# byteowlz/kokorox

Measured on AMD Instinct MI355X. Metric: real-time factor (audio-s/wall-s), 24 kHz, batch=64, higher is better.
Workload: dtype f32 in / out, f32 accumulate; products on split operands: f16f8 (a_hi b_hi on f16 MFMAs, the cross terms a_lo b_hi + a_hi b_lo of the 7 / 11-tap convs on e4m3 scaled MFMAs: ~17 significant bits per product; every other conv f16x3: ~22) -- wider than the bf16 BASELINE configs[2] names, inside the 1e-; 1 GPU; batch=64/GPU synthetic 128-phoneme utterances (T=130), durations pinned 3,3,3,4 -> F=422 frames = 10.55 s each, noise on, inputs in HBM; batch_per_gpu=64, frames=422, parallelism=utterance-sharded x1, one-time weight broadcast

## Files before the change

kokorox_amd/build.py:

```python
from __future__ import annotations

import os
import subprocess
import sys

HERE = os.path.dirname(os.path.abspath(__file__))
CSRC = os.path.join(HERE, "csrc")
LIB_DIR = os.path.join(HERE, "lib")
LIB_PATH = os.path.join(LIB_DIR, "libkokorox_hip.so")
TEST_LIB_PATH = os.path.join(LIB_DIR, "libkokorox_hip_test.so")
TEST_SOURCES = ["test_hooks.hip"]
SOURCES = ["conv_plan.hip", "conv_call.hip", "conv_mfma.hip", "conv_f16x3.hip", "conv_f16x3_da.hip", "conv_f16x3_da_p1.hip", "conv_f16x3_da_w2.hip", "conv_f16x3_da_s16.hip", "conv_f16x3_da_f8.hip", "conv_f16x3_da_pre.hip", "conv_f16x3_pre.hip", "conv_f16x3_dapn.hip", "conv_f16x3_dag.hip", "kernels_misc.hip", "request_kernels.hip", "model.hip", "model_forward.hip", "model_host.hip", "api.hip", "dispatcher.hip", "onnx_import.cpp", "kxw_file.cpp",
           "host_request.cpp", "host_pool.cpp"]
HEADERS = ["kx_common.h", "kx_error.h", "host_request.h", "conv_epilogue.h", "conv_f16x3_common.h"]
_PUB = os.path.join("..", "..", "include", "kokorox_hip.h")
_PUB_TEST = os.path.join("..", "..", "include", "kokorox_hip_test.h")
_MODEL_H = ["model.h", "kxw_file.h", "onnx_import.h"]
EXTRA_DEPS = {"model.hip": [*_MODEL_H, _PUB], "model_forward.hip": [*_MODEL_H, _PUB], "model_host.hip": [*_MODEL_H, "host_pool.h", _PUB],
              "host_pool.cpp": ["host_pool.h"], "host_request.cpp": ["resample_taps.h", "kweight_coefs.h", "truepeak_taps.h"], "request_kernels.hip": ["resample_taps.h", "kweight_coefs.h", "truepeak_taps.h"], "conv_call.hip": _MODEL_H, "api.hip": [*_MODEL_H, "kx_handle.h", "api_guard.h", "check_device.h", _PUB],
              "dispatcher.hip": [*_MODEL_H, "kx_handle.h", "dispatcher_core.h", _PUB],
              "test_hooks.hip": [*_MODEL_H, "kx_handle.h", "api_guard.h", "check_device.h", _PUB, _PUB_TEST], "onnx_import.cpp": ["onnx_import.h"],
              "kxw_file.cpp": ["kxw_file.h", "onnx_import.h"], "conv_f16x3_da_p1.hip": ["conv_f16x3_da.hip"], "conv_f16x3_da_w2.hip": ["conv_f16x3_da.hip"], "conv_f16x3_da_s16.hip": ["conv_f16x3_da.hip"], "conv_f16x3_da_f8.hip": ["conv_f16x3_da.hip"], "conv_f16x3_da_pre.hip": ["conv_f16x3_da.hip"]}
FLAGS = ["-O3", "--offload-arch=gfx950", "-fPIC", "-std=c++17", "-Wall", "-Wno-unused-result"]


def _hipcc() -> str:
    for cand in (os.environ.get("HIPCC"), "/opt/rocm/bin/hipcc", "hipcc"):
        if cand and (os.path.isabs(cand) and os.path.exists(cand) or not os.path.isabs(cand)):
            return cand
    return "hipcc"


def _newer(target: str, deps) -> bool:
    if not os.path.exists(target):
        return False
    t = os.path.getmtime(target)
    return all(os.path.getmtime(d) <= t for d in deps)


LAST_BUILD = {"compiled": [], "reused": [], "linked": False}


def build_library(force: bool = False, verbose: bool = False) -> str:
    LAST_BUILD["compiled"], LAST_BUILD["reused"], LAST_BUILD["linked"] = [], [], False
    os.makedirs(LIB_DIR, exist_ok=True)
    hdrs = [os.path.join(CSRC, h) for h in HEADERS]
    objs, test_objs, jobs = [], [], []
    for src in SOURCES + TEST_SOURCES:
        s = os.path.join(CSRC, src)
        o = os.path.join(LIB_DIR, os.path.splitext(src)[0] + ".o")
        (test_objs if src in TEST_SOURCES else objs).append(o)
        if force or not _newer(o, [s] + hdrs + [os.path.join(CSRC, d) for d in EXTRA_DEPS.get(src, [])]):
            flags = [f for f in FLAGS if not f.startswith("--offload-arch")] if src.endswith(".cpp") else FLAGS
            jobs.append([_hipcc(), *flags, "-c", s, "-o", o])
            LAST_BUILD["compiled"].append(src)
        else:
            LAST_BUILD["reused"].append(src)
    if jobs:
        from concurrent.futures import ThreadPoolExecutor

        def run(cmd):
            if verbose:
                print(" ".join(cmd), file=sys.stderr)
            subprocess.run(cmd, check=True)

        with ThreadPoolExecutor(max_workers=min(4, len(jobs))) as ex:
            list(ex.map(run, jobs))
    if force or not _newer(LIB_PATH, objs):
        cmd = [_hipcc(), "--offload-arch=gfx950", "-shared", "-fPIC", *objs, "-lpthread", "-o", LIB_PATH]
        if verbose:
            print(" ".join(cmd), file=sys.stderr)
        subprocess.run(cmd, check=True)
        LAST_BUILD["linked"] = True
    if force or not _newer(TEST_LIB_PATH, test_objs + [LIB_PATH]):
        cmd = [_hipcc(), "--offload-arch=gfx950", "-shared", "-fPIC", *test_objs, "-L" + LIB_DIR, "-lkokorox_hip", "-Wl,-rpath,$ORIGIN",
               "-lpthread", "-o", TEST_LIB_PATH]
        if verbose:
            print(" ".join(cmd), file=sys.stderr)
        subprocess.run(cmd, check=True)
    return LIB_PATH


if __name__ == "__main__":
    print(build_library(force="--force" in sys.argv, verbose=True))
```

kokorox_amd/csrc/conv_f16x3.hip:

```cpp
#include "conv_f16x3_common.h"

namespace kx {

template <int BM, int BN, int WM, int WN, int ACT, int TK, bool PF, int VT>
__global__ __launch_bounds__(WM * WN * 64, (WM * WN == 8) ? 4 : ((BM / WM / 32) * (BN / WN / 32) > 6 ? 2 : 3))
void conv1d_f16x3_kernel(const ConvArgs a) {
    constexpr int MT = BM / WM / 32;
    constexpr int NT = BN / WN / 32;
    constexpr int NWV = WM * WN;
    static_assert((NWV == 4 || NWV == 8) && MT >= 1 && NT >= 1, "4 or 8 waves per workgroup");
    static_assert(VT == 1 || (VT <= TK && PF), "virtual taps need TK >= VT and the prefetching build");
    extern __shared__ __attribute__((aligned(16))) unsigned char smem16[];

    const int tid = threadIdx.x;
    const int lane = tid & 63;
    const int wave = __builtin_amdgcn_readfirstlane(tid >> 6);
    const int wm = wave / WN, wn = wave % WN;
    const int r = lane & 31, h = lane >> 5;
    const int b = blockIdx.z, ct = blockIdx.y;
    int tile_x = blockIdx.x;
    if (a.xcd_swizzle && gridDim.x >= 16) {
        const int nx = gridDim.x;
        const int off = (int)(((long)nx * (blockIdx.y + (long)gridDim.y * blockIdx.z)) & 7);
        const int cls = (blockIdx.x + off) & 7;
// ... 300 lines not shown

template <int BM, int BN, int WM, int WN, int ACT, int TK, bool PF, int VT = 1>
static void launch_inst16_pf(const ConvArgs& a, int B, int max_cols, hipStream_t s) {
    static DynLdsLimit lds_limit;
    auto kern = conv1d_f16x3_kernel<BM, BN, WM, WN, ACT, TK, PF, VT>;
    const int XW = (BN - 1) * a.stride + (a.K - 1) * a.dil + 1;
    const int XWp = PF ? ((VT > 1) ? 128 : BN + 128) : ((XW + 3) & ~3);
    KX_REQUIRE(!PF || (a.stride == 1 && XW <= XWp), "conv1d f16x3: the prefetching build needs stride 1 and a window <= BN + 128");
    const size_t lds = 16 * ((size_t)2 * TK * 4 * BM + (size_t)VT * 4 * XWp);
    KX_REQUIRE(lds <= 160 * 1024, "conv1d f16x3: LDS tile too large for this k/stride");
    KX_REQUIRE(VT == 1 || (a.K == 1 && a.stride == 1 && XW <= 128), "conv1d f16x3: virtual taps need a k=1 GEMM");
    lds_limit.ensure(reinterpret_cast<const void*>(kern), lds);
    dim3 grid((max_cols + BN - 1) / BN, (a.Cout + BM - 1) / BM, a.merge_T > 0 ? 1 : B);
    KX_REQUIRE(grid.x > 0 && grid.y > 0 && grid.y < 65536 && B > 0 && B < 65536, "conv1d f16x3: bad grid");
    KX_REQUIRE(a.merge_T == 0 || (PF && a.K == 1 && a.stride == 1 && a.pad == 0 && !a.in_up2 && !a.nmean &&
                                  a.store != ST_UPSCATTER && !a.stat_part),
               "conv1d f16x3: merged columns need a plain k=1 GEMM");
    hipLaunchKernelGGL(kern, grid, dim3(WM * WN * 64), lds, s, a);
    KX_HIP(hipGetLastError());
}

template <int BM, int BN, int WM, int WN, int ACT>
static void launch_inst16_act(const ConvPlan& p, const ConvArgs& a, int B, hipStream_t s) {
    if (p.pf)
        launch_inst16_pf<BM, BN, WM, WN, ACT, 3, true>(a, B, p.cols, s);
    else
        launch_inst16_pf<BM, BN, WM, WN, ACT, 3, false>(a, B, p.cols, s);
}

template <int BM, int BN, int WM, int WN>
static void launch_inst16(const ConvPlan& p, const ConvArgs& a, int B, hipStream_t s) {
    if (p.act == ACT_SNAKE)
        launch_inst16_act<BM, BN, WM, WN, ACT_SNAKE>(p, a, B, s);
    else if (p.act == ACT_LEAKY)
        launch_inst16_act<BM, BN, WM, WN, ACT_LEAKY>(p, a, B, s);
    else
        launch_inst16_act<BM, BN, WM, WN, ACT_NONE>(p, a, B, s);
}

static void launch_lds(const ConvPlan& p, const ConvArgs& a, int B, hipStream_t s) {
    if (p.vt > 1) {
        KX_REQUIRE(p.bm == 128 && p.bn == 128 && p.pf && p.act != ACT_SNAKE && (p.vt == 2 || p.vt == 3), "conv1d f16x3: no such virtual-tap form");
        if (p.vt == 3) {
            if (p.act == ACT_LEAKY)
                launch_inst16_pf<128, 128, 2, 2, ACT_LEAKY, 3, true, 3>(a, B, p.cols, s);
            else
                launch_inst16_pf<128, 128, 2, 2, ACT_NONE, 3, true, 3>(a, B, p.cols, s);
        } else {
            if (p.act == ACT_LEAKY)
                launch_inst16_pf<128, 128, 2, 2, ACT_LEAKY, 2, true, 2>(a, B, p.cols, s);
            else
                launch_inst16_pf<128, 128, 2, 2, ACT_NONE, 2, true, 2>(a, B, p.cols, s);
        }
        return;
    }
    const int bm = p.bm, bn = p.bn, wm = p.wm, wn = p.wn;
    if (bm == 128 && bn == 128 && wm == 4 && wn == 1)
        launch_inst16<128, 128, 4, 1>(p, a, B, s);
    else if (bm == 128 && bn == 128 && wm == 2 && wn == 2)
        launch_inst16<128, 128, 2, 2>(p, a, B, s);
    else if (bm == 128 && bn == 256 && wm == 2 && wn == 2)
        launch_inst16<128, 256, 2, 2>(p, a, B, s);
    else if (bm == 64 && bn == 256 && wm == 1 && wn == 4)
        launch_inst16<64, 256, 1, 4>(p, a, B, s);
    else if (bm == 32 && bn == 256 && wm == 1 && wn == 4)
        launch_inst16<32, 256, 1, 4>(p, a, B, s);
    else
        throw Error(1, "conv1d f16x3: no such LDS-DMA form");
}

void launch_conv(const ConvPlan& p, const ConvArgs& a, int B, hipStream_t s) {
    if (p.form == FORM_F32) {
        launch_conv1d(a, p.bm, B, p.cols, s);
        return;
    }
    KX_REQUIRE(a.n_chunks16 == (a.Cin + CK16 - 1) / CK16 && a.w16 != nullptr, "conv1d f16x3: weights not packed");
    KX_REQUIRE(a.epi != EPI_GELU_NEW || p.vt > 1 || p.form == FORM_DAG || p.form == FORM_DAGN,
               "conv1d f16x3: gelu epilogue exists only for k=1 GEMMs with >= 48 input channels");
    KX_REQUIRE(p.merged == (a.merge_T > 0), "conv1d f16x3: merged columns do not match the plan");
    if (p.cols <= 0) return;
    switch (p.form) {
        case FORM_LDS: launch_lds(p, a, B, s); return;
        case FORM_DAG:
        case FORM_DAGN: launch_conv1d_f16x3_dag(p, a, B, s); return;
        case FORM_DAPN: launch_conv1d_f16x3_dapn(a, B, p.cols, s); return;
        case FORM_DA_PRE: launch_conv16_da_pre(p, a, B, s); return;
        case FORM_DA_S16: launch_conv16_da_s16(p, a, B, s); return;
        case FORM_DA_F8: launch_conv16_da_f8(p, a, B, s); return;
        case FORM_DA:
            if (p.p1) {
                launch_conv16_da_p1(p, a, B, s);
                return;
            }
            [[fallthrough]];
        case FORM_DA_W2:
            if (p.form == FORM_DA_W2)
                launch_conv16_da_w2(p, a, B, s);
            else
                launch_conv16_da(p, a, B, s);
            return;
    }
    throw Error(1, "conv1d: unknown kernel form");
}

size_t packed_conv16_halves(int rows, int Cin, int K, int BM) {
    const size_t tiles = (rows + BM - 1) / BM, chunks = (Cin + CK16 - 1) / CK16;
    return tiles * chunks * K * 4 * BM * 8;
}

__global__ void absmax_kernel(const float* p, long n, unsigned* out) {
    unsigned m = 0u;
    for (long i = blockIdx.x * (long)blockDim.x + threadIdx.x; i < n; i += (long)gridDim.x * blockDim.x) {
        const unsigned u = __float_as_uint(p[i]) & 0x7fffffffu;
        m = u > m ? u : m;
    }
    for (int o = 32; o > 0; o >>= 1) {
        const unsigned u = (unsigned)__shfl_down((int)m, o);
        m = u > m ? u : m;
    }
    if ((threadIdx.x & 63) == 0) atomicMax(out, m);
}

float device_absmax(const float* p, long n, hipStream_t s) {
    unsigned* d;
    KX_HIP(hipMalloc((void**)&d, 4));
    KX_HIP(hipMemsetAsync(d, 0, 4, s));
    const int blocks = (int)((n + 255) / 256 < 1024 ? (n + 255) / 256 : 1024);
    hipLaunchKernelGGL(absmax_kernel, dim3(blocks), dim3(256), 0, s, p, n, d);
    unsigned hbits = 0;
    KX_HIP(hipMemcpyAsync(&hbits, d, 4, hipMemcpyDeviceToHost, s));
    KX_HIP(hipStreamSynchronize(s));
    KX_HIP(hipFree(d));
    float f;
    memcpy(&f, &hbits, 4);
    return f;
}

int pick_weight_shift(float absmax) {
    if (!(absmax > 0.f) || !std::isfinite(absmax)) return 0;
    int e;
    frexpf(absmax, &e);
    int ws = 12 - e;
    if (ws < -8) ws = -8;
    if (ws > 24) ws = 24;
    return ws;
}

__global__ void pack_conv16_kernel(PackSrc src, _Float16* dst, int Cout, int Cin, int K, int BM, float wscale,
                                   long total_pairs) {
    const int n_chunks = (Cin + CK16 - 1) / CK16;
    for (long e = blockIdx.x * (long)blockDim.x + threadIdx.x; e < total_pairs; e += (long)gridDim.x * blockDim.x) {
        long q = e;
        const int j8 = q % 8; q /= 8;
        const int m = q % BM; q /= BM;
        const int hh = q % 2; q /= 2;
        const int tap = q % K; q /= K;
        const int ch = q % n_chunks; q /= n_chunks;
        const int co = (int)q * BM + m, ci = ch * CK16 + hh * 8 + j8;
        float v = 0.f;
        if (co < Cout && ci < Cin) {
            int rr = co;
            const float* p = src.p[0];
            if (rr >= src.rows[0]) { rr -= src.rows[0]; p = src.p[1];
                if (rr >= src.rows[1]) { rr -= src.rows[1]; p = src.p[2]; } }
            v = p[((long)rr * Cin + ci) * K + tap] * wscale;
        }
// ... 109 lines not shown
```

kokorox_amd/csrc/conv_plan.hip:

```cpp
#include "kx_common.h"

namespace kx {

static bool da_eligible(int BM, int K, int dil, int stride, bool merged) {
    return BM == 128 && stride == 1 && !merged && (K - 1) * dil + 256 <= 384;
}

static bool f8_taps(int K, int dil) { return (K == 11 || K == 7 || K == 3) && (K - 1) * dil <= 64; }

static bool s16_shape(int BM, int K, int dil, int stride, int act, int n_chunks16, bool merged, int pmode) {
    const bool taps = K == 11 || (K == 7 && dil == 1) || (pmode == 2 && f8_taps(K, dil));
    return BM == 128 && stride == 1 && !merged && pmode != 1 && act == ACT_SNAKE && taps && (K - 1) * dil <= 64 && n_chunks16 >= 2 &&
           (n_chunks16 & 1) == 0;
}

bool conv16_f8_layer(int BM, int rows, int K, int n_chunks16) {
    return BM == 128 && f8_taps(K, 1) && (K != 3 || rows <= 256) && n_chunks16 >= 2 && (n_chunks16 & 1) == 0;
}

ConvPlan conv_plan(const ConvLaunch& c) {
    ConvPlan p{};
    p.bm = c.BM;
    p.act = c.act;
    p.vt = 1;
    p.cols = c.cols;
    const bool stats = c.stats && c.store == ST_NORMAL && !c.accum;
    auto set_stats = [&](int stat_cols) {
        if (!stats) return;
        p.stat_cols = stat_cols;
        p.stat_tiles = (p.cols + p.bn - 1) / p.bn * (p.bn / stat_cols);
    };
    if (c.mode == CONV_F32) {
        p.form = FORM_F32;
        p.bn = c.BM == 128 ? 128 : 256;
        set_stats(64);
        return p;
    }
    const int route = c.force & 3;
    const int pmode = c.prec1 ? 1 : (c.f8 ? 2 : 0);

    const bool pre_form = c.stride == 1 && c.K >= 2 && !c.in_up2 && c.act != ACT_SNAKE && !c.prec1 &&
                          da_eligible(c.BM, c.K, c.dil, c.stride, false);
    p.pre = (c.mode == CONV_F16X3 || c.mode == CONV_F16F8) && c.image && pre_form && (c.image == 2 || c.rows >= 512);

    p.merged = c.B > 1 && c.K == 1 && c.stride == 1 && c.pad == 0 && !c.in_up2 && !c.norm && c.store != ST_UPSCATTER && !c.stats &&
               c.merge_T > 0 && c.merge_T <= 512;
    if (p.merged) p.cols = c.B * c.merge_T;

    if (c.BM != 128) {
        p.form = FORM_LDS;
        p.bn = 256;
        p.wm = 1;
        p.wn = 4;
        p.pf = c.stride == 1 && (c.K - 1) * c.dil <= 128;
        set_stats(64);
        return p;
    }

    if (c.K == 1 && c.stride == 1 && !stats && !c.in_up2 && c.n_chunks16 >= 3 && c.act != ACT_SNAKE) {
        const long tiles = (long)((p.cols + 127) / 128) * ((c.rows + 127) / 128);
        if (route != FORCE_LDS && !c.norm && c.store != ST_UPSCATTER) {
            const long wgs = tiles * (p.merged ? 1 : c.B);
            const bool narrow_ok = (c.x_bs * c.B + 16L * c.x_ld) * 4 < (1L << 31);
            p.form = narrow_ok && 2 * wgs <= c.cus ? FORM_DAGN : FORM_DAG;
            p.bn = p.form == FORM_DAGN ? 32 : 128;
            return p;
        }
        p.form = FORM_LDS;
        p.bn = 128;
        p.wm = 2;
        p.wn = 2;
        p.pf = 1;
        p.vt = tiles > 2L * c.cus ? 2 : 3;
        return p;
    }

    const bool da = route != FORCE_LDS && da_eligible(c.BM, c.K, c.dil, c.stride, p.merged);
    const bool small = (long)((p.cols + 255) / 256) * ((c.rows + 127) / 128) * c.B < 256;
    if (route != FORCE_LDS && !(c.force & FORCE_NO_S16) && s16_shape(c.BM, c.K, c.dil, c.stride, c.act, c.n_chunks16, p.merged, pmode)) {
        p.form = pmode == 2 ? FORM_DA_F8 : FORM_DA_S16;
        p.kt = c.K;
        p.bn = small && route != FORCE_DA ? 128 : 192;
        set_stats(64);
    } else if (!da || (route != FORCE_DA && c.cols <= 160 && !stats)) {
        p.form = FORM_LDS;
        const bool short_seq = c.cols <= 160 && !stats;
        p.bn = !short_seq && !small ? 256 : 128;
        p.wm = !short_seq && small ? 4 : 2;
        p.wn = !short_seq && small ? 1 : 2;
        p.pf = c.stride == 1 && (c.K - 1) * c.dil <= 128;
        set_stats(p.bn / p.wn);
    } else {
        p.bn = small && route != FORCE_DA ? 128 : 256;
        set_stats(128);
        const bool w64 = (c.K - 1) * c.dil <= 64;
        if (p.pre) {
            const bool narrow = p.bn == 128 && !c.prec1 && c.rows % 32 == 0 && c.K <= 12 && c.epi == EPI_NONE &&
                                (c.store == ST_NORMAL || c.store == ST_UPSCATTER) && (long)c.n_chunks16 * c.K < 5000;
            p.form = narrow ? FORM_DAPN : FORM_DA_PRE;
            p.act = ACT_NONE;
            p.kt = c.K == 3 && w64 ? 3 : 0;
        } else {
            const bool unrolled = w64 && ((c.act == ACT_SNAKE && (c.K == 11 || c.K == 7 || c.K == 3)) || (c.act == ACT_LEAKY && c.K == 3));
            p.kt = unrolled ? c.K : 0;
            p.p1 = c.prec1 != 0;
            p.bf = c.prec1 == 2;
            p.form = unrolled && p.bn == 256 && !c.prec1 && !(c.force & FORCE_DA_4X1) ? FORM_DA_W2 : FORM_DA;
        }
    }
    const bool flat_form = p.form != FORM_LDS;
    p.flat_bn = flat_form && c.B > 1 && p.cols > 0 ? p.bn : 0;
    return p;
}

}
```

kokorox_amd/csrc/kx_common.h:

```cpp
#pragma once
#include <hip/hip_runtime.h>

#include <cmath>
#include <cstdint>
#include <cstring>
#include <cstdio>
#include <stdexcept>
#include <string>
#include <vector>

#include <atomic>
#include <mutex>

#include "host_request.h"
#include "kx_error.h"

namespace kx {

constexpr int KX_MAX_DEVICES = 64;

struct DynLdsLimit {
    std::atomic<size_t> limit[KX_MAX_DEVICES];
    std::mutex mu;
    DynLdsLimit() {
// ... 21 lines not shown

struct LenMap {
    const int* lens;
    int mul, add;
};

constexpr int CONV_CK = 8;

enum ConvAct { ACT_NONE = 0, ACT_LEAKY = 1, ACT_SNAKE = 2 };
enum ConvStore { ST_NORMAL = 0, ST_TMAJOR = 1, ST_UPSCATTER = 2 };
enum ConvEpi { EPI_NONE = 0, EPI_GELU_NEW = 1 };

struct ConvArgs {
    const float* x;
    long x_bs;
    int x_ld;
    int Cin;
    LenMap in_len;
    LenMap out_len;
    const float* w;
    const float* bias;
    const float* nmean;
    const float* nscale;
    const float* nshift;
    int n_bs;
    int act;
    float slope;
    const float* alpha;
    int K, dil, stride, pad;
    int in_up2;
    int Cout;
    int n_chunks;
    float* y;
    long y_bs;
    int y_ld;
    const float* resid;
    long r_bs;
    int r_ld;
    int accum;
    float out_mul;
    float out_div;
    int epi;
    int store;
    int up_s, up_pad, up_off, up_reflect, up_cout;
    const void* w16;
    const void* w16b;
    const void* w8x;
    int epi_stream;
    int n_chunks16;
    float w_unscale;
    float x_prescale;
    int merge_T;
    int merge_B;
    float2* stat_part;
    int stat_tiles;
    int xcd_swizzle;
    int ws_force;
    unsigned long long* stamps;
    int prec1;
    int dephase_cycles, dephase_mode;
    int dbg;
    const int* tile_prefix;
    int flat_ny;
    int flat_B;
    int flat_tiles_host, flat_bn_host;
    const void* x16;
    long x16_bs;
    int x16_ld;
};

enum ConvMode { CONV_F32 = 0, CONV_F16X3 = 1, CONV_F16X3_LDS = 2, CONV_F16X3_DA = 3, CONV_F16 = 4, CONV_BF16 = 5, CONV_F16F8 = 6 };
enum ConvForm {
    FORM_F32 = 0,
    FORM_LDS,
    FORM_DAG,
    FORM_DAGN,
    FORM_DA,
    FORM_DA_W2,
    FORM_DA_S16,
    FORM_DA_F8,
    FORM_DA_PRE,
    FORM_DAPN,
};
enum ConvForce { FORCE_LDS = 1, FORCE_DA = 2, FORCE_DA_4X1 = 4, FORCE_NO_S16 = 8 };

struct ConvLaunch {
    int mode;
    int prec1;
    int f8;
    int BM, rows, n_chunks16, K, dil, stride, pad, act, in_up2, store, accum, epi;
    int norm;
    int stats;
    int image;
    int merge_T;
    long x_bs;
    int x_ld;
    int B, cols;
    int cus;
    int force;
};
struct ConvPlan {
    int form;
    int bm, act, kt, wm, wn, vt, pf, p1, bf;
    int bn;
    int cols;
    int merged;
    int pre;
    int stat_cols, stat_tiles;
    int flat_bn;
};
ConvPlan conv_plan(const ConvLaunch& c);
bool conv16_f8_layer(int BM, int rows, int K, int n_chunks16);
void launch_conv(const ConvPlan& p, const ConvArgs& a, int B, hipStream_t s);
int conv16_cu_count();
int cu_count_override();

size_t conv16_pre_image_bytes(int Cin, int x_ld);
void launch_split_image(const ConvArgs& a, int B, int Lmax, void* img, long img_bs, hipStream_t s);

void launch_tile_prefix(LenMap len, int extra, int bn, int B, int* out, hipStream_t s);

inline int conv_pick_bm(int rows) { return rows >= 128 ? 128 : (rows > 32 ? 64 : 32); }

void launch_conv1d(const ConvArgs& a, int BM, int B, int max_cols, hipStream_t s);

struct PackSrc {
    const float* p[3];
    int rows[3];
};
void launch_pack_conv(const PackSrc& src, float* dst, int Cout, int Cin, int K, int BM, hipStream_t s);
void launch_pack_convT(const float* w, float* dst, int Cin, int Cout, int s, int BM, hipStream_t s_);
size_t packed_conv_floats(int rows, int Cin, int K, int BM);

void launch_conv16_da(const ConvPlan& p, const ConvArgs& a, int B, hipStream_t s);
void launch_conv16_da_p1(const ConvPlan& p, const ConvArgs& a, int B, hipStream_t s);
void launch_conv16_da_w2(const ConvPlan& p, const ConvArgs& a, int B, hipStream_t s);
void launch_conv16_da_s16(const ConvPlan& p, const ConvArgs& a, int B, hipStream_t s);
void launch_conv16_da_f8(const ConvPlan& p, const ConvArgs& a, int B, hipStream_t s);
void launch_conv16_da_pre(const ConvPlan& p, const ConvArgs& a, int B, hipStream_t s);
void launch_conv1d_f16x3_dapn(const ConvArgs& a, int B, int max_cols, hipStream_t s);
void launch_conv1d_f16x3_dag(const ConvPlan& p, const ConvArgs& a, int B, hipStream_t s);
size_t packed_conv16_halves(int rows, int Cin, int K, int BM);
float device_absmax(const float* p, long n, hipStream_t s);
int pick_weight_shift(float absmax);
void launch_pack_conv16(const PackSrc& src, void* dst, int Cout, int Cin, int K, int BM, float wscale, hipStream_t s);
void launch_pack_convT16(const float* w, void* dst, int Cin, int Cout, int sd, int BM, float wscale, hipStream_t s);
void launch_image_to_bf16(const void* w16, void* dst, size_t n_halves, hipStream_t s);
size_t packed_conv8x_bytes(int rows, int Cin, int K);
void launch_pack_conv8x(const void* w16, void* dst, int rows, int Cin, int K, hipStream_t s);

void launch_vec_add(const float* a, const float* b, float* out, int n, hipStream_t s);
void launch_transpose_whh(const float* whh, float* out, hipStream_t s);

void launch_albert_embed(const int64_t* ids, long ids_stride, const float* word, const float* type0,
                         const float* pos, float* out, long bs, int ld, const int* lens, int B, int Tmax,
                         int n_vocab, unsigned* bad_id, hipStream_t s);
void launch_embed(const int64_t* ids, long ids_stride, const float* table, int C, float* out, long bs, int ld,
                  const int* lens, int B, int Tmax, int n_vocab, unsigned* bad_id, hipStream_t s);

enum LnMode { LN_PLAIN = 0, LN_AFFINE = 1, LN_ADA = 2 };
void launch_layernorm_ch(const float* x, float* y, long bs, int ld, int C, LenMap len, int B, int Lmax,
                         float eps, int mode, const float* g, const float* be, int g_bs, float leaky,
                         hipStream_t s);

void launch_attention(const float* qkv, long bs, int ld, float* ctx, long cbs, int cld, const int* lens, int B,
                      int Tmax, hipStream_t s);

struct FcDesc {
    const float* w;
    const float* b;
    int n_out;
    int style_off;
    long out_off;
};
void launch_style_fc(const FcDesc* d_desc, int n_desc, const float* styles, float* out, long out_bs, int B,
                     hipStream_t s);

constexpr int STAT_RAW_TILES = 0;
void launch_stats_finalize(const float2* part, int tiles, int cols_per_tile, int C, LenMap len, int B, const float* gb,
                           long gb_bs, float* mean, float* scale, float* shift, int n_bs, hipStream_t s);
void launch_in_stats(const float* x, long bs, int ld, int C, LenMap len, int B, const float* gb, long gb_bs,
                     float* mean, float* scale, float* shift, int n_bs, float2* raw_out, hipStream_t s);

void launch_diag_stats(const float* x, long bs, int ld, int C, LenMap len, int B, int Lmax, const float* nmean,
                       const float* nscale, const float* nshift, int n_bs, float* out3, hipStream_t s);

void launch_style_mix(const float* table, int n_voices, const int* voice_ids, const float* weights, int max_mix,
                      const int* rows, const int* kinds, float* styles, int B, hipStream_t s);

struct OutputTables {
    PackReq* req;
    long* cum;
    JoinRow* join;
    MarkRow* mark;
    LevelSpec* level;
    uint32_t* peak;
    LoudSpec* loud;
    double* hops;
    double* loud_pow;
    uint32_t* tpeak;
};
void launch_output_plan(const float* audio, long audio_ld, const int* dur, const int* lens, const OutputPlan& plan,
                        const OutputTables& t, float* d_y, void* d_packed, hipStream_t s);
void launch_pack_plan(const float* audio, long audio_ld, const OutputPlan& plan, const OutputTables& t, float* d_y, void* out,
                      hipStream_t s);
void launch_token_marks(const int* dur, const int* lens, const OutputPlan& plan, const OutputTables& t, void* marks, hipStream_t s);
void launch_edge_durations(const int* dur, const int* lens, int* edges, int B, hipStream_t s);
void* host_out_alloc(size_t bytes);
void host_out_free(void* p);
void host_out_share(void* base, void* const* parts, int n);
size_t host_out_live_bytes();
void launch_fill_style_rows(float* dst, long bs, int ld, int row0, const float* styles, int style_off,
                            const int* lens, int B, int Tmax, hipStream_t s);
void launch_copy_rows(const float* src, long sbs, int sld, float* dst, long dbs, int dld, int rows, LenMap len,
                      int B, int Lmax, hipStream_t s);

void launch_lstm(const float* gx, long gx_bs, int gx_ld, const float* whhT, float* y, long y_bs, int y_ld,
                 LenMap len, int B, unsigned long long* xchg, unsigned* err_word, hipStream_t s,
                 unsigned* epoch_state = nullptr);
size_t lstm_exchange_bytes(int B);
void lstm_set_parts(int n);
void lstm_set_test_fault(int on);

void launch_duration(const float* logits, long bs, int ld, const float* speeds, int n_speed, const int* lens,
// ... 23 lines not shown
```

kokorox_amd/hip_koko.py:

```python
from __future__ import annotations

import ctypes as C
import os
from typing import List, Optional, Sequence

import numpy as np

_HERE = os.path.dirname(os.path.abspath(__file__))
LIB_PATH = os.path.join(_HERE, "lib", "libkokorox_hip.so")

PACK_F32_MONO, PACK_F32_STEREO, PACK_PCM16_MONO = 0, 1, 2
PACK_WAV_F32, PACK_WAV16_BASE64 = 3, 4
PACK_MULAW, PACK_ALAW = 8, 9
PACK_RATE_24000, PACK_RATE_8000, PACK_RATE_16000, PACK_RATE_48000 = 0x000, 0x100, 0x200, 0x300
RATE_HZ = {0: 24000, 1: 8000, 2: 16000, 3: 48000}
RESAMPLE_MAX_TAPS = 145
JOIN_TRIM_HEAD, JOIN_TRIM_TAIL, JOIN_TRIM_INNER = 1, 2, 4
JOIN_DTYPE = np.dtype([("flags", "<u4"), ("keep_ms", "<i4"), ("pause_ms", "<i4"), ("fade_ms", "<i4")])
JOIN_NONE = (0, 0, 0, 0)
LEVEL_GAIN, LEVEL_NORMALIZE, LEVEL_CEILING = 0, 1, 2
LEVEL_DTYPE = np.dtype([("mode", "<u4"), ("gain", "<f4"), ("peak", "<f4")])
LEVEL_PLAIN = (LEVEL_GAIN, 1.0, 0.0)
PEAK_TRUE = 0x100
LOUDNESS_MEASURE, LOUDNESS_NORMALIZE = 0, 1
# ... 761 lines not shown
        try:
            raw = C.string_at(out, nb.value)
            if marks:
                if (mk.value or 0) % 8 != 0 or (mk.value or 0) < out.value + nb.value:
                    raise KokoroxHipError(3, "marks are not 8-byte aligned behind the body")
                m = np.frombuffer(C.string_at(mk, 8 * n_mk.value), dtype=np.int64).copy()
        finally:
            self._lib.kx_free_packed(out)
        res = (_decode_packed(raw, fmt), m) if marks else (_decode_packed(raw, fmt),)
        res = res + (lv_out,) if level is not None else res
        res = res + (ld_out,) if loudness is not None else res
        return res if len(res) > 1 else res[0]

    def stats(self):
        a, b, c = C.c_int64(0), C.c_int64(0), C.c_int64(0)
        self._lib.kx_dispatcher_stats(self._d, C.byref(a), C.byref(b), C.byref(c))
        per = (C.c_int64 * len(self._models))()
        self._lib.kx_dispatcher_model_batches(self._d, per, len(self._models))
        rp, rt = C.c_int64(0), C.c_int64(0)
        self._lib.kx_dispatcher_failures(self._d, C.byref(rp), C.byref(rt))
        hl = (C.c_int32 * len(self._models))()
        mf, rq = C.c_int64(0), C.c_int64(0)
        self._lib.kx_dispatcher_health(self._d, hl, len(self._models), C.byref(mf), C.byref(rq))
        return {"requests": a.value, "batches": b.value, "max_batch": c.value, "batches_per_model": list(per),
                "replayed_requests": rp.value, "retried_batches": rt.value, "healthy": [int(v) for v in hl],
                "failed_models": mf.value, "requeued_requests": rq.value}

    def close(self):
        if getattr(self, "_d", None):
            self._lib.kx_dispatcher_destroy(self._d)
            self._d = None

    def __del__(self):
        try:
            self.close()
        except Exception:
            pass


def import_onnx(onnx_path: str, out_path: str) -> str:
    lib = load_library()
    err = C.create_string_buffer(2048)
    rc = lib.kx_import_onnx(os.fsencode(onnx_path), os.fsencode(out_path), err, len(err))
    if rc != KX_OK:
        raise KokoroxHipError(rc, err.value.decode(errors="replace"))
    return out_path


def _err_call(fn, *args):
    err = C.create_string_buffer(512)
    rc = fn(*args, err, len(err))
    if rc != 0:
        raise KokoroxHipError(rc, err.value.decode())


CONV_F32, CONV_F16X3, CONV_F16F8 = 0, 1, 6
STFT_ONNX, STFT_TORCH = 0, 1


def conv1d(x, w, bias=None, stride=1, pad=0, dil=1, transposed=False, act=0, slope=0.0, alpha=None, norm=None,
           device=0, mode=None, pre=False):
    lib = load_test_library()
    if mode is None:
        mode = CONV_F32 if os.environ.get("KOKOROX_CONV", "") == "f32" else CONV_F16X3
    x, w = _f32(x), _f32(w)
    B, Cin, L = x.shape
    k = w.shape[2]
    if transposed:
        Cout = w.shape[1]
        Lout = (L - 1) * stride - 2 * pad + k
    else:
        Cout = w.shape[0]
        Lout = (L + 2 * pad - dil * (k - 1) - 1) // stride + 1
    y = np.zeros((B, Cout, Lout), dtype=np.float32)
    bias, alpha, norm = _f32(bias), _f32(alpha), _f32(norm)
    _err_call(lib.kx_test_conv1d, device, _ptr(x), B, Cin, L, _ptr(w), _ptr(bias), Cout, k, stride, pad, dil,
              1 if transposed else 0, act, float(slope), _ptr(alpha), _ptr(norm), _ptr(y), Lout, mode | (0x100 if pre else 0))
    return y


CONV_LAUNCH_FIELDS = ("mode", "prec1", "f8", "BM", "rows", "n_chunks16", "K", "dil", "stride", "pad", "act", "in_up2", "store", "accum",
                      "epi", "norm", "stats", "image", "merge_T", "x_bs", "x_ld", "B", "cols", "cus", "force")
CONV_PLAN_FIELDS = ("form", "bm", "act", "kt", "wm", "wn", "vt", "pf", "p1", "bf", "bn", "cols", "merged", "pre", "stat_cols",
                    "stat_tiles", "flat_bn")
CONV_FORMS = ("F32", "LDS", "DAG", "DAGN", "DA", "DA_W2", "DA_S16", "DA_F8", "DA_PRE", "DAPN")


def conv_plan(**launch):
    lib = load_test_library()
    unknown = set(launch) - set(CONV_LAUNCH_FIELDS)
    assert not unknown, unknown
    src = np.array([int(launch.get(f, 0)) for f in CONV_LAUNCH_FIELDS], dtype=np.int64)
    out = np.zeros(len(CONV_PLAN_FIELDS), dtype=np.int64)
    _err_call(lib.kx_test_conv_plan, _ptr(src), len(src), _ptr(out), len(out))
    plan = dict(zip(CONV_PLAN_FIELDS, (int(v) for v in out)))
    plan["form"] = CONV_FORMS[plan["form"]]
    return plan


def conv_transpose(x, w, bias=None, stride=6, act=1, slope=0.1, resid=None, up_off=0, mode=1, pre=False, device=0):
    lib = load_test_library()
    x, w = _f32(x), _f32(w)
    B, Cin, L = x.shape
    Cout, k = w.shape[1], w.shape[2]
    assert k == 2 * stride
    pad = (k - stride) // 2
    Lout = (L - 1) * stride - 2 * pad + k
    y = np.zeros((B, Cout, Lout + (1 if up_off else 0)), dtype=np.float32)
    _err_call(lib.kx_test_conv_transpose, device, _ptr(x), B, Cin, L, _ptr(w), _ptr(_f32(bias)), Cout, stride, act, float(slope),
              _ptr(_f32(resid)), 1 if up_off else 0, _ptr(y), mode | (0x100 if pre else 0))
    return y


def conv1d_epilogue(x, w, bias=None, pad=0, dil=1, resid=None, y_init=None, out_mul=1.0, out_div=1.0, want_stats=False,
                    mode=1, device=0):
    lib = load_test_library()
    x, w = _f32(x), _f32(w)
    B, Cin, L = x.shape
    Cout, _, k = w.shape
    Lout = L + 2 * pad - dil * (k - 1)
    y = np.zeros((B, Cout, Lout), dtype=np.float32) if y_init is None else _f32(y_init).copy()
    st = np.zeros((B, Cout, 2), dtype=np.float32) if want_stats else None
    _err_call(lib.kx_test_conv1d_epilogue, device, _ptr(x), B, Cin, L, _ptr(w), _ptr(_f32(bias)), Cout, k, pad, dil,
              _ptr(_f32(resid)), 0 if y_init is None else 1, float(out_mul), float(out_div), _ptr(y), _ptr(st), mode)
    return (y, st) if want_stats else y


def conv1d_full(x, w, bias=None, pad=0, dil=1, act=0, slope=0.0, alpha=None, norm=None, resid=None, y_init=None,
                out_mul=1.0, out_div=1.0, want_stats=False, lens=None, pad_ld=False, flat=False, mode=1, device=0, pre=False):
    lib = load_test_library()
    x, w = _f32(x), _f32(w)
    B, Cin, L = x.shape
    Cout, _, k = w.shape
    Lout = L + 2 * pad - dil * (k - 1)
    y = np.zeros((B, Cout, Lout), dtype=np.float32) if y_init is None else _f32(y_init).copy()
    st = np.zeros((B, Cout, 2), dtype=np.float32) if want_stats else None
    ln = None if lens is None else np.ascontiguousarray(lens, dtype=np.int32)
    _err_call(lib.kx_test_conv1d_full, device, _ptr(x), B, Cin, L, _ptr(ln), (1 if pad_ld else 0) | (2 if flat else 0), _ptr(w), _ptr(_f32(bias)),
              Cout, k, pad, dil, act, float(slope), _ptr(_f32(alpha)), _ptr(_f32(norm)), _ptr(_f32(resid)),
              0 if y_init is None else 1, float(out_mul), float(out_div), _ptr(y), _ptr(st), mode | (0x100 if pre else 0))
    return (y, st) if want_stats else y


def conv1d_opts(x, w, bias=None, pad=0, dil=1, act=0, slope=0.0, alpha=None, norm=None, resid=None, y_init=None,
                out_mul=1.0, out_div=1.0, want_stats=False, lens=None, pad_ld=False, flat=False, mode=1, device=0, pre=False,
                in_up2=False, epi=0, merged=False, tmajor=False, prec1=0, act_shift=0, epi_stream=False, want_norm=None,
                up_stride=0, stride=1, len_in=None, len_out=None, up_off=False, view=False):
    lib = load_test_library()
    x, w = _f32(x), _f32(w)
    B, Cin, L = x.shape
    Cout, _, k = w.shape
    Lout = ((2 * L if in_up2 else L) + 2 * pad - dil * (k - 1) - 1) // stride + 1
    if up_stride:
        Cout = w.shape[1]
        assert k == 2 * up_stride
        Lout = (L - 1) * up_stride - 2 * ((k - up_stride) // 2) + k + (1 if up_off else 0)
    shape = (B, Lout, Cout) if tmajor else (B, Cout, Lout)
    y = np.zeros(shape, dtype=np.float32) if y_init is None else _f32(y_init).copy()
    st = np.zeros((B, Cout, 2), dtype=np.float32) if want_stats else None
    ln = None if lens is None else np.ascontiguousarray(lens, dtype=np.int32)
    opts = [in_up2, epi, merged, tmajor, prec1, act_shift, epi_stream, up_stride]
    if stride != 1 or len_in is not None or len_out is not None or up_off or view:
        opts += [stride, *(len_in or (0, 0)), *(len_out or (0, 0)), up_off, view]
    opts = np.array(opts, dtype=np.int32)
    gb = _f32(want_norm)
    planes = None if gb is None else np.zeros((3, B, Cout), dtype=np.float32)
    assert gb is None or gb.shape == (B, 2 * Cout)
# ... 325 lines not shown
```

Measured before the change: 6801 x realtime.

## Add deep-pipelined DAG kernel for 1-tap GEMMs at low tile counts

Adds a new 1x1 conv (k=1 GEMM) kernel that register-prefetches six weight chunks and double-buffers split-f16 input tiles in LDS. It overlaps the global loads and the activation/split transform of the next super-chunk with the current MFMAs, using scheduling barriers. The planner routes FORM_DAG launches to it when the workgroup count is at most two per CU, with force flags to override. The aim is to hide load latency in deep-Cin GEMMs that have few tiles, at the cost of higher register pressure and a new code path.

```diff
diff --git a/kokorox_amd/build.py b/kokorox_amd/build.py
--- a/kokorox_amd/build.py
+++ b/kokorox_amd/build.py
@@ -10,7 +10,7 @@
 LIB_PATH = os.path.join(LIB_DIR, "libkokorox_hip.so")
 TEST_LIB_PATH = os.path.join(LIB_DIR, "libkokorox_hip_test.so")
 TEST_SOURCES = ["test_hooks.hip"]
-SOURCES = ["conv_plan.hip", "conv_call.hip", "conv_mfma.hip", "conv_f16x3.hip", "conv_f16x3_da.hip", "conv_f16x3_da_p1.hip", "conv_f16x3_da_w2.hip", "conv_f16x3_da_s16.hip", "conv_f16x3_da_f8.hip", "conv_f16x3_da_pre.hip", "conv_f16x3_pre.hip", "conv_f16x3_dapn.hip", "conv_f16x3_dag.hip", "kernels_misc.hip", "request_kernels.hip", "model.hip", "model_forward.hip", "model_host.hip", "api.hip", "dispatcher.hip", "onnx_import.cpp", "kxw_file.cpp",
+SOURCES = ["conv_plan.hip", "conv_call.hip", "conv_mfma.hip", "conv_f16x3.hip", "conv_f16x3_da.hip", "conv_f16x3_da_p1.hip", "conv_f16x3_da_w2.hip", "conv_f16x3_da_s16.hip", "conv_f16x3_da_f8.hip", "conv_f16x3_da_pre.hip", "conv_f16x3_pre.hip", "conv_f16x3_dapn.hip", "conv_f16x3_dag.hip", "conv_f16x3_dagd.hip", "kernels_misc.hip", "request_kernels.hip", "model.hip", "model_forward.hip", "model_host.hip", "api.hip", "dispatcher.hip", "onnx_import.cpp", "kxw_file.cpp",
            "host_request.cpp", "host_pool.cpp"]
 HEADERS = ["kx_common.h", "kx_error.h", "host_request.h", "conv_epilogue.h", "conv_f16x3_common.h"]
 _PUB = os.path.join("..", "..", "include", "kokorox_hip.h")
diff --git a/kokorox_amd/csrc/conv_f16x3.hip b/kokorox_amd/csrc/conv_f16x3.hip
--- a/kokorox_amd/csrc/conv_f16x3.hip
+++ b/kokorox_amd/csrc/conv_f16x3.hip
@@ -406,6 +406,11 @@
     switch (p.form) {
         case FORM_LDS: launch_lds(p, a, B, s); return;
         case FORM_DAG:
+            if (p.deep) {
+                launch_conv1d_f16x3_dagd(a, B, p.cols, s);
+                return;
+            }
+            [[fallthrough]];
         case FORM_DAGN: launch_conv1d_f16x3_dag(p, a, B, s); return;
         case FORM_DAPN: launch_conv1d_f16x3_dapn(a, B, p.cols, s); return;
         case FORM_DA_PRE: launch_conv16_da_pre(p, a, B, s); return;
diff --git a/kokorox_amd/csrc/conv_f16x3_dagd.hip b/kokorox_amd/csrc/conv_f16x3_dagd.hip
--- /dev/null
+++ b/kokorox_amd/csrc/conv_f16x3_dagd.hip
@@ -0,0 +1,243 @@
+#include "conv_f16x3_common.h"
+#include <type_traits>
+
+#ifndef KX_DAGD_BUFS
+#define KX_DAGD_BUFS 2
+#endif
+
+namespace kx {
+
+template <int I, int N, class F>
+__device__ __forceinline__ void static_for_d(F&& f) {
+    if constexpr (I < N) {
+        f(std::integral_constant<int, I>{});
+        static_for_d<I + 1, N>(f);
+    }
+}
+
+constexpr int BUF_WORD3 = 0x00020000;
+
+template <int ACT>
+__global__ __launch_bounds__(256, 2) void conv1d_f16x3_dagd_kernel(const ConvArgs a) {
+    constexpr int BM = 128, BN = 128, NT = 4, VT = 3, NB = KX_DAGD_BUFS, XD = NB - 1;
+    static_assert(NB >= 2 && NB <= 3, "LDS buffers: two workgroups of NB x 24 KiB must fit a CU");
+    constexpr int XWp = BN;
+    constexpr int XIMG = 4 * XWp;
+    constexpr int XBUF = VT * XIMG;
+    constexpr int tap_units = 4 * BM;
+    extern __shared__ __attribute__((aligned(16))) unsigned char smem16[];
+    uint4* Xs = reinterpret_cast<uint4*>(smem16);
+
+    const int tid = threadIdx.x;
+    const int lane = tid & 63;
+    const int wave = __builtin_amdgcn_readfirstlane(tid >> 6);
+    const int r = lane & 31, h = lane >> 5;
+    const int b = blockIdx.z;
+    int tile_x = blockIdx.x, ct = blockIdx.y;
+    {
+        const int nx = gridDim.x, ny = gridDim.y, N = nx * ny;
+        const int l = blockIdx.x + nx * blockIdx.y;
+        int lp = l;
+        if (a.xcd_swizzle && N >= 16) {
+            const int off = (int)(((long)N * blockIdx.z) & 7);
+            const int cls = (l + off) & 7;
+            int start = 0;
+            for (int c = 0; c < cls; ++c) {
+                const int first = (c - off) & 7;
+                start += first < N ? (N - first + 7) >> 3 : 0;
+            }
+            lp = start + (l >> 3);
+        }
+        if (a.xcd_swizzle) {
+            tile_x = lp / ny;
+            ct = lp - tile_x * ny;
+        }
+    }
+    const int t0 = tile_x * BN;
+    const bool merged = a.merge_T > 0;
+    const int Lin = merged ? a.merge_B * a.merge_T : a.in_len.lens[b] * a.in_len.mul + a.in_len.add;
+    const int Lout = merged ? Lin : a.out_len.lens[b] * a.out_len.mul + a.out_len.add;
+    const int ncols = Lout;
+    if (t0 >= ncols) return;
+
+    const int n_chunks = a.n_chunks16;
+    const int n_super = (n_chunks + VT - 1) / VT;
+
+    f32x16 acc[1][NT];
+#pragma unroll
+    for (int j = 0; j < NT; ++j)
+#pragma unroll
+        for (int e = 0; e < 16; ++e) acc[0][j][e] = 0.f;
+
+    const int g = wave & 1, jb = wave >> 1;
+    float raw[2][VT][8];
+    unsigned xoff;
+    bool pok;
+    {
+        const int p = t0 - a.pad + lane + 64 * jb;
+        if (merged) {
+            const int pc = p < Lin ? (p < 0 ? 0 : p) : Lin - 1;
+            const int bb = pc / a.merge_T, tt = pc - bb * a.merge_T;
+            pok = p >= 0 && p < Lin && tt < a.in_len.lens[bb];
+            xoff = (unsigned)(int)((long)bb * a.x_bs + tt);
+        } else {
+            pok = p >= 0 && p < Lin;
+            xoff = (unsigned)(p < 0 ? 0 : (p >= Lin ? Lin - 1 : p));
+        }
+    }
+    const float* xbase = merged ? a.x : a.x + (long)b * a.x_bs;
+    const unsigned x_bytes = (unsigned)(((merged ? (long)(a.merge_B - 1) * a.x_bs : 0L) + (long)a.Cin * a.x_ld) * 4);
+    const __amdgpu_buffer_rsrc_t xres = __builtin_amdgcn_make_buffer_rsrc(const_cast<float*>(xbase), 0, (int)x_bytes, BUF_WORD3);
+    const int xvo = (int)(xoff * 4u);
+    const int cmax_in = a.Cin - 1;
+    const int row_bytes = a.x_ld * 4;
+    auto load_pair = [&](float (&rw)[VT][8], const int vt, const int c2, int sc) __attribute__((always_inline)) {
+#pragma unroll
+        for (int q = 0; q < 2; ++q) {
+            const int c = 2 * c2 + q;
+            const int ci = (sc * VT + vt) * CK16 + g * 8 + c;
+            const int so = __builtin_amdgcn_readfirstlane((ci < cmax_in ? ci : cmax_in) * row_bytes);
+            rw[vt][c] = __builtin_bit_cast(float, __builtin_amdgcn_raw_buffer_load_b32(xres, xvo, so, 0));
+        }
+    };
+    const float keep = pok ? a.x_prescale : 0.f;
+    auto xform_pair = [&](const float (&rw)[VT][8], const int vt, const int c2, uint4* Xb, int sc) __attribute__((always_inline)) {
+        float y2[2];
+#pragma unroll
+        for (int q = 0; q < 2; ++q) {
+            const int c = 2 * c2 + q;
+            const float y = in_act<ACT>(rw[vt][c], a.slope, 1.f, 1.f);
+            y2[q] = y * (((sc * VT + vt) * CK16 + g * 8 + c <= cmax_in) ? keep : 0.f);
+        }
+        unsigned hp, lp;
+        split_pair(y2[0], y2[1], hp, lp);
+        const int u = lane + 64 * jb;
+        unsigned* Xw = reinterpret_cast<unsigned*>(Xb + vt * XIMG);
+        Xw[((0 * 2 + g) * XWp + u) * 4 + c2] = hp;
+        Xw[((1 * 2 + g) * XWp + u) * 4 + c2] = lp;
+    };
+
+    const uint4* wtile = reinterpret_cast<const uint4*>(a.w16) + (long)ct * n_chunks * tap_units;
+    const __amdgpu_buffer_rsrc_t wres =
+        __builtin_amdgcn_make_buffer_rsrc(const_cast<uint4*>(wtile), 0, n_chunks * tap_units * 16, BUF_WORD3);
+    const int wvo = (h * BM + wave * 32 + r) * 16;
+    using u32x4 = __attribute__((ext_vector_type(4))) unsigned;
+    auto load_A = [&](int s, u32x4& a_hi, u32x4& a_lo) __attribute__((always_inline)) {
+        const int sc = s < n_chunks ? s : n_chunks - 1;
+        const int so = __builtin_amdgcn_readfirstlane(sc * (tap_units * 16));
+        a_hi = __builtin_amdgcn_raw_buffer_load_b128(wres, wvo, so, 0);
+        a_lo = __builtin_amdgcn_raw_buffer_load_b128(wres, wvo, so + 2 * BM * 16, 0);
+    };
+    u32x4 ahs[6], als[6];
+    static_for_d<0, 6>([&](auto sc_) __attribute__((always_inline)) {
+        constexpr int s = decltype(sc_)::value;
+        load_A(s, ahs[s], als[s]);
+    });
+    __builtin_amdgcn_sched_barrier(0);
+#pragma unroll
+    for (int u = 0; u < 2; ++u)
+#pragma unroll
+        for (int vt = 0; vt < VT; ++vt)
+#pragma unroll
+            for (int c2 = 0; c2 < 4; ++c2) load_pair(raw[u], vt, c2, u);
+    __builtin_amdgcn_sched_barrier(0);
+    static_for_d<0, XD>([&](auto jc) __attribute__((always_inline)) {
+        constexpr int j = decltype(jc)::value;
+#pragma unroll
+        for (int vt = 0; vt < VT; ++vt)
+#pragma unroll
+            for (int c2 = 0; c2 < 4; ++c2) {
+                xform_pair(raw[j & 1], vt, c2, Xs + j * XBUF, j);
+                __builtin_amdgcn_sched_barrier(0);
+                load_pair(raw[j & 1], vt, c2, j + 2);
+            }
+    });
+    __syncthreads();
+
+    int cur = 0, wr = XD;
+    half8 fh[3], fl[3];
+    auto load_tile = [&](int vt, int n, half8& fhx, half8& flx) __attribute__((always_inline)) {
+        const uint4* xt = Xs + cur * XBUF + vt * XIMG + h * XWp + r + n * 32;
+        fhx = *reinterpret_cast<const half8*>(xt);
+        flx = *reinterpret_cast<const half8*>(xt + 2 * XWp);
+    };
+    load_tile(0, 0, fh[0], fl[0]);
+    load_tile(0, 1, fh[1], fl[1]);
+    constexpr int TILES = NT * VT;
+    auto super_chunk = [&](auto uc, const int sc) __attribute__((always_inline)) {
+        constexpr int U = decltype(uc)::value, RS = (U + XD) & 1;
+        static_for_d<0, TILES>([&](auto ic) __attribute__((always_inline)) {
+            constexpr int i = decltype(ic)::value;
+            constexpr int t = i / NT, n = i % NT, sl = 3 * U + t;
+            constexpr int e = i % 3, ip = i + 2, e2 = ip % 3;
+            const half8 ah = __builtin_bit_cast(half8, ahs[sl]), al = __builtin_bit_cast(half8, als[sl]);
+            if constexpr (ip < TILES) load_tile(ip / NT, ip % NT, fh[e2], fl[e2]);
+            __builtin_amdgcn_sched_barrier(0);
+            acc[0][n] = __builtin_amdgcn_mfma_f32_32x32x16_f16(al, fh[e], acc[0][n], 0, 0, 0);
+            acc[0][n] = __builtin_amdgcn_mfma_f32_32x32x16_f16(ah, fl[e], acc[0][n], 0, 0, 0);
+            acc[0][n] = __builtin_amdgcn_mfma_f32_32x32x16_f16(ah, fh[e], acc[0][n], 0, 0, 0);
+            if constexpr (i >= TILES / 2) {
+                constexpr int p0 = 2 * (i - TILES / 2);
+                xform_pair(raw[RS], p0 / 4, p0 % 4, Xs + wr * XBUF, sc + XD);
+                xform_pair(raw[RS], (p0 + 1) / 4, (p0 + 1) % 4, Xs + wr * XBUF, sc + XD);
+#pragma unroll
+                for (int k3 = 0; k3 < 3; ++k3) {
+                    __builtin_amdgcn_sched_group_barrier(0x008, 1, 0);
+                    __builtin_amdgcn_sched_group_barrier(0x002, 11, 0);
+                }
+                __builtin_amdgcn_sched_barrier(0);
+                load_pair(raw[RS], p0 / 4, p0 % 4, sc + XD + 2);
+                load_pair(raw[RS], (p0 + 1) / 4, (p0 + 1) % 4, sc + XD + 2);
+            }
+            __builtin_amdgcn_sched_barrier(0);
+            if constexpr (n == NT - 1) {
+                load_A((sc + 2) * VT + t, ahs[sl], als[sl]);
+                __builtin_amdgcn_sched_barrier(0);
+            }
+        });
+        __builtin_amdgcn_fence(__ATOMIC_RELEASE, "workgroup");
+        __builtin_amdgcn_s_barrier();
+        __builtin_amdgcn_fence(__ATOMIC_ACQUIRE, "workgroup");
+        cur = cur + 1 == NB ? 0 : cur + 1;
+        wr = wr + 1 == NB ? 0 : wr + 1;
+        load_tile(0, 0, fh[0], fl[0]);
+        load_tile(0, 1, fh[1], fl[1]);
+    };
+    int sc = 0;
+    for (; sc + 1 < n_super; sc += 2) {
+        super_chunk(std::integral_constant<int, 0>{}, sc);
+        super_chunk(std::integral_constant<int, 1>{}, sc + 1);
+    }
+    if (sc < n_super) super_chunk(std::integral_constant<int, 0>{}, sc);
+
+    conv_store_tile<1, NT, EPI_ROWS, true>(a, acc, a.w_unscale, b, ct * BM + wave * 32, t0, r, h, ncols, Lout, tile_x, nullptr);
+}
+
+template <int ACT>
+static void launch_dagd_inst(const ConvArgs& a, int B, int max_cols, hipStream_t s) {
+    auto kern = conv1d_f16x3_dagd_kernel<ACT>;
+    constexpr size_t lds = 16 * (size_t)KX_DAGD_BUFS * 3 * 4 * 128;
+    static DynLdsLimit lim;
+    lim.ensure(reinterpret_cast<const void*>(kern), lds);
+    dim3 grid((max_cols + 127) / 128, (a.Cout + 127) / 128, a.merge_T > 0 ? 1 : B);
+    KX_REQUIRE(grid.x > 0 && grid.y > 0 && grid.y < 65536 && B > 0 && B < 65536, "conv1d f16x3 dag deep: bad grid");
+    hipLaunchKernelGGL(kern, grid, dim3(256), lds, s, a);
+    KX_HIP(hipGetLastError());
+}
+
+void launch_conv1d_f16x3_dagd(const ConvArgs& a, int B, int max_cols, hipStream_t s) {
+    KX_REQUIRE(a.K == 1 && a.stride == 1 && !a.stat_part && !a.in_up2 && a.n_chunks16 >= 3 && a.act != ACT_SNAKE && a.nmean == nullptr &&
+                   a.store != ST_UPSCATTER,
+               "conv1d f16x3 dag deep: launch not eligible");
+    KX_REQUIRE(a.n_chunks16 == (a.Cin + CK16 - 1) / CK16 && a.w16 != nullptr, "conv1d f16x3 dag deep: weights not packed");
+    KX_REQUIRE(a.pad == 0, "conv1d f16x3 dag deep: a 1-tap GEMM has no padding");
+    if (max_cols <= 0) return;
+    const long x_bytes = ((a.merge_T > 0 ? (long)(a.merge_B - 1) * a.x_bs : 0L) + (long)a.Cin * a.x_ld) * 4;
+    KX_REQUIRE(x_bytes < (1L << 31) && (long)a.n_chunks16 * 8192 < (1L << 31), "conv1d f16x3 dag deep: input beyond 2 GiB");
+    if (a.act == ACT_LEAKY)
+        launch_dagd_inst<ACT_LEAKY>(a, B, max_cols, s);
+    else
+        launch_dagd_inst<ACT_NONE>(a, B, max_cols, s);
+}
+
+}
diff --git a/kokorox_amd/csrc/conv_plan.hip b/kokorox_amd/csrc/conv_plan.hip
--- a/kokorox_amd/csrc/conv_plan.hip
+++ b/kokorox_amd/csrc/conv_plan.hip
@@ -1,4 +1,8 @@
 #include "kx_common.h"
+
+#ifndef KX_DAGD_MAX_TILES_PER_CU
+#define KX_DAGD_MAX_TILES_PER_CU 2
+#endif
 
 namespace kx {
 
@@ -62,8 +66,12 @@
         if (route != FORCE_LDS && !c.norm && c.store != ST_UPSCATTER) {
             const long wgs = tiles * (p.merged ? 1 : c.B);
             const bool narrow_ok = (c.x_bs * c.B + 16L * c.x_ld) * 4 < (1L << 31);
-            p.form = narrow_ok && 2 * wgs <= c.cus ? FORM_DAGN : FORM_DAG;
+            const bool deep_ok = ((p.merged ? c.x_bs * c.B : 0L) + 16L * c.n_chunks16 * c.x_ld) * 4 < (1L << 31);
+            const bool force_deep = deep_ok && (c.force & FORCE_DEEP) && !(c.force & FORCE_SHALLOW);
+            p.form = narrow_ok && 2 * wgs <= c.cus && !force_deep ? FORM_DAGN : FORM_DAG;
             p.bn = p.form == FORM_DAGN ? 32 : 128;
+            p.deep = p.form == FORM_DAG && deep_ok && !(c.force & FORCE_SHALLOW) &&
+                     (force_deep || wgs <= (long)KX_DAGD_MAX_TILES_PER_CU * c.cus);
             return p;
         }
         p.form = FORM_LDS;
diff --git a/kokorox_amd/csrc/kx_common.h b/kokorox_amd/csrc/kx_common.h
--- a/kokorox_amd/csrc/kx_common.h
+++ b/kokorox_amd/csrc/kx_common.h
@@ -127,7 +127,7 @@
     FORM_DA_PRE,
     FORM_DAPN,
 };
-enum ConvForce { FORCE_LDS = 1, FORCE_DA = 2, FORCE_DA_4X1 = 4, FORCE_NO_S16 = 8 };
+enum ConvForce { FORCE_LDS = 1, FORCE_DA = 2, FORCE_DA_4X1 = 4, FORCE_NO_S16 = 8, FORCE_DEEP = 16, FORCE_SHALLOW = 32 };
 
 struct ConvLaunch {
     int mode;
@@ -153,6 +153,7 @@
     int pre;
     int stat_cols, stat_tiles;
     int flat_bn;
+    int deep;
 };
 ConvPlan conv_plan(const ConvLaunch& c);
 bool conv16_f8_layer(int BM, int rows, int K, int n_chunks16);
@@ -185,6 +186,7 @@
 void launch_conv16_da_pre(const ConvPlan& p, const ConvArgs& a, int B, hipStream_t s);
 void launch_conv1d_f16x3_dapn(const ConvArgs& a, int B, int max_cols, hipStream_t s);
 void launch_conv1d_f16x3_dag(const ConvPlan& p, const ConvArgs& a, int B, hipStream_t s);
+void launch_conv1d_f16x3_dagd(const ConvArgs& a, int B, int max_cols, hipStream_t s);
 size_t packed_conv16_halves(int rows, int Cin, int K, int BM);
 float device_absmax(const float* p, long n, hipStream_t s);
 int pick_weight_shift(float absmax);
diff --git a/kokorox_amd/hip_koko.py b/kokorox_amd/hip_koko.py
--- a/kokorox_amd/hip_koko.py
+++ b/kokorox_amd/hip_koko.py
@@ -867,7 +867,7 @@
 CONV_LAUNCH_FIELDS = ("mode", "prec1", "f8", "BM", "rows", "n_chunks16", "K", "dil", "stride", "pad", "act", "in_up2", "store", "accum",
                       "epi", "norm", "stats", "image", "merge_T", "x_bs", "x_ld", "B", "cols", "cus", "force")
 CONV_PLAN_FIELDS = ("form", "bm", "act", "kt", "wm", "wn", "vt", "pf", "p1", "bf", "bn", "cols", "merged", "pre", "stat_cols",
-                    "stat_tiles", "flat_bn")
+                    "stat_tiles", "flat_bn", "deep")
 CONV_FORMS = ("F32", "LDS", "DAG", "DAGN", "DA", "DA_W2", "DA_S16", "DA_F8", "DA_PRE", "DAPN")
 
 
```

Result: no change. 6821 x realtime (median of 6 runs) (+0.3%).
